# PaddlePaddle/PaddleRobotics

Measured on AMD Instinct MI355X. Metric: env-steps/sec, 4096 A1 quadrupeds; 1/2/4/8-GPU scaling, higher is better.
Workload: dtype f32

## Files before the change

paddlerobotics_amd/csrc/etg_core16.h:

```cpp
#pragma once

#include <type_traits>

#include "etg_core.h"

namespace etg {

template <class Ctx, class = void> struct sweep_stream_ : std::false_type {};
template <class Ctx> struct sweep_stream_<Ctx, std::void_t<decltype(Ctx::kSweepStream)>> : std::bool_constant<Ctx::kSweepStream> {};
template <class Ctx, class... Args> ETG_HD void run_sweep_stream_(const Ctx& c, Args&&... args) { c.pgs_body_stream(args...); }
template <class Ctx, class = void> struct gram_mfma_ : std::false_type {};
template <class Ctx> struct gram_mfma_<Ctx, std::void_t<decltype(Ctx::kGramMfma)>> : std::bool_constant<Ctx::kGramMfma> {};

template <class F> struct State16 {
  V3<F> p;
  F qx, qy, qz, qw;
  V3<F> wb, vb;
  F q, qd;
  F lam;
  F contact;
  F energy;
  int sweeps;
};

template <class F, class Ctx> ETG_HD State16<F> load_state16(const Ctx& c, const float* base, const float* leg) {
  State16<F> L;
  L.p = {c.ld_env(base, BS_PX), c.ld_env(base, BS_PY), c.ld_env(base, BS_PZ)};
  L.qx = c.ld_env(base, BS_QX); L.qy = c.ld_env(base, BS_QY); L.qz = c.ld_env(base, BS_QZ); L.qw = c.ld_env(base, BS_QW);
  L.wb = {c.ld_env(base, BS_WX), c.ld_env(base, BS_WY), c.ld_env(base, BS_WZ)};
  L.vb = {c.ld_env(base, BS_VX), c.ld_env(base, BS_VY), c.ld_env(base, BS_VZ)};
  const F mj = c.jointf();
  L.q = mj * c.ld_joint(leg, LG_Q);
  L.qd = mj * c.ld_joint(leg, LG_QD);
  L.lam = c.ld_quad(leg, LG_LAM);
  L.contact = c.ld_legf(leg, LG_CONTACT);
// ... 252 lines not shown
    nwo = nw;
    const V t1w = {it1 * (one - nwx * nwx), -(it1 * (nwx * nwy)), -(it1 * (nwx * nwz))};
    const V t2w = {zero, it1 * nwz, -(it1 * nwy)};
    const auto s2 = c.sub_is(2);
    const V dw = {sel_(s1, t1w.x, sel_(s2, t2w.x, nw.x)), sel_(s1, t1w.y, sel_(s2, t2w.y, nw.y)), sel_(s1, t1w.z, sel_(s2, t2w.z, nw.z))};
    dn = {Rw.r0.x * nw.x + Rw.r1.x * nw.y + Rw.r2.x * nw.z, Rw.r0.y * nw.x + Rw.r1.y * nw.y + Rw.r2.y * nw.z,
          Rw.r0.z * nw.x + Rw.r1.z * nw.y + Rw.r2.z * nw.z};
    dir = {Rw.r0.x * dw.x + Rw.r1.x * dw.y + Rw.r2.x * dw.z, Rw.r0.y * dw.x + Rw.r1.y * dw.y + Rw.r2.y * dw.z,
           Rw.r0.z * dw.x + Rw.r1.z * dw.y + Rw.r2.z * dw.z};
  }
  auto act = phi < F(K.margin);
  const F rowf = (bodies ? one : mj) * sel_(act, one, zero) * live;
  V rc = pc - rad * dn;
  V k1 = cross(xax, rc - g.o1), k2 = cross(g.yax, rc - g.o2), k3 = cross(g.yax, rc - g.o3);
  if (knee) {
    if (Ctx::kFlat) dir = {sel_(s3, dn.x, dir.x), sel_(s3, dn.y, dir.y), sel_(s3, dn.z, dir.z)};
    const V rn = rad * dn;
    const V a12 = q12 - s12 * rn, a3 = ps_ - rn;
    const V b1 = cross(xax, a12 - s12 * g.o1), b2 = cross(g.yax, a12 - s12 * g.o2), b3 = bw1 * cross(g.yax, a3 - g.o3);
    k1 = {sel_(s3, b1.x, k1.x), sel_(s3, b1.y, k1.y), sel_(s3, b1.z, k1.z)};
    k2 = {sel_(s3, b2.x, k2.x), sel_(s3, b2.y, k2.y), sel_(s3, b2.z, k2.z)};
    k3 = {sel_(s3, b3.x, k3.x), sel_(s3, b3.y, k3.y), sel_(s3, b3.z, k3.z)};
  }
  const bool anyb = bodies && c.any_body((rowf * f3) > F(0.5f));
  F Jl0 = rowf * dot(dir, k1), Jl1 = rowf * dot(dir, k2), Jl2 = rowf * dot(dir, k3);
  F HJ0 = Hi11 * Jl0 + Hi12 * Jl1 + Hi13 * Jl2;
  F HJ1 = Hi12 * Jl0 + Hi22 * Jl1 + Hi23 * Jl2;
  F HJ2 = Hi13 * Jl0 + Hi23 * Jl1 + Hi33 * Jl2;
  W Jb = rowf * W{cross(rc, dir), dir};
  W G = Jb - (HJ0 * Fj[0] + HJ1 * Fj[1] + HJ2 * Fj[2]);
  F g6[6] = {G.a.x, G.a.y, G.a.z, G.l.x, G.l.y, G.l.z};
  fwd6(s, g6);
  const W sqv = {{sq[0], sq[1], sq[2]}, {sq[3], sq[4], sq[5]}};
  const W Zv = cmul(W{{g6[0], g6[1], g6[2]}, {g6[3], g6[4], g6[5]}}, sqv);
  F Z[6] = {Zv.a.x, Zv.a.y, Zv.a.z, Zv.l.x, Zv.l.y, Zv.l.z};
  c.phase(5);
  F lam = rowf * sel_(s0, F(K.warmstart), sel_(c.sub_is(3), F(K.warmstart_b), F(K.warmstart_t))) * L.lam;
  F hj[3] = {HJ0, HJ1, HJ2};
  constexpr bool gram = gram_mfma_<Ctx>::value;
  F A[4][3];
  F Akz[4] = {zero, zero, zero, zero};
  if constexpr (gram) {
    c.dpp_ready4(hj, &lam);
    typename Ctx::gram_t Af[4];
    c.gram16(Af, Z, Z);
#pragma unroll
    for (int lp = 0; lp < 4; lp++) {
// ... 127 lines not shown
    for (int k = 0; k < 6; k++) Z2[k] = comp(Z2v, k);
    const V vc2 = vbs + cross(wbs, rc2) + qs0 * kb1 + qs1 * kb2 + qs2 * kb3;
    u2s = rowf2 * dot(dir2, vc2);
    c.dpp_ready(Z2, 6);
    c.dpp_ready(hj2, 3);
    if constexpr (gram) {
      typename Ctx::gram_t Bf[4];
      c.gram16(Bf, Z, Z2);
#pragma unroll
      for (int lp = 0; lp < 4; lp++)
#pragma unroll
        for (int e = 0; e < 4; e++) BA[lp][e] = Bf[lp][e];
    }
#pragma unroll
    for (int lp = 0; lp < 4; lp++) {
#pragma unroll
      for (int e = 0; e < 4; e++) {
        if constexpr (!gram) {
          BA[lp][e] = c.rbcast(Z[0], 4 * lp + e) * Z2[0];
#pragma unroll
          for (int k = 1; k < 6; k++) c.fmac_rbcast(BA[lp][e], Z[k], Z2[k], 4 * lp + e);
        }
      }
#pragma unroll
      for (int t = 0; t < 2; t++) {
        BB[lp][t] = c.rbcast(Z2[0], 4 * lp + 1 + t) * Z2[0];
        AT[lp][t] = c.rbcast(Z2[0], 4 * lp + 1 + t) * Z[0];
#pragma unroll
        for (int k = 1; k < 6; k++) {
          c.fmac_rbcast(BB[lp][t], Z2[k], Z2[k], 4 * lp + 1 + t);
          c.fmac_rbcast(AT[lp][t], Z2[k], Z[k], 4 * lp + 1 + t);
        }
      }
    }
    F oa[4], ob[2], ot[2];
#pragma unroll
    for (int e = 0; e < 4; e++) oa[e] = c.qb(hj[0], e) * Jb0 + c.qb(hj[1], e) * Jb1 + c.qb(hj[2], e) * Jb2_;
#pragma unroll
    for (int t = 0; t < 2; t++) {
      ob[t] = c.qb(hj2[0], 1 + t) * Jb0 + c.qb(hj2[1], 1 + t) * Jb1 + c.qb(hj2[2], 1 + t) * Jb2_;
      ot[t] = c.qb(hj2[0], 1 + t) * Jl0 + c.qb(hj2[1], 1 + t) * Jl1 + c.qb(hj2[2], 1 + t) * Jl2;
    }
#pragma unroll
    for (int lp = 0; lp < 4; lp++) {
#pragma unroll
      for (int e = 0; e < 4; e++) BA[lp][e] = BA[lp][e] + ownl[lp] * oa[e];
#pragma unroll
      for (int t = 0; t < 2; t++) { BB[lp][t] = BB[lp][t] + ownl[lp] * ob[t]; AT[lp][t] = AT[lp][t] + ownl[lp] * ot[t]; }
    }
    F Add2 = hj2[0] * Jb0 + hj2[1] * Jb1 + hj2[2] * Jb2_;
    Add2 = Add2 + dot(Z2v, Z2v);
    iA2 = sel_(rowf2 > F(0.5f), rcp_(Add2), zero);
#pragma unroll
    for (int lp = 0; lp < 4; lp++) {
#pragma unroll
      for (int e = 0; e < 4; e++) { if (b_lds) c.slotb_st(4 * lp + e, BA[lp][e]); else sb[4 * lp + e] = BA[lp][e]; }
#pragma unroll
      for (int t = 0; t < 2; t++) {
        if (b_lds) { c.slotb_st(16 + 2 * lp + t, BB[lp][t]); c.slotb_st(24 + 2 * lp + t, AT[lp][t]); }
        else { sb[16 + 2 * lp + t] = BB[lp][t]; sb[24 + 2 * lp + t] = AT[lp][t]; }
      }
    }
    c.phase_p(12);
  }
  F sgn = zero, lamq = zero, iAq = zero, c0q = zero;
  F zj[6] = {zero, zero, zero, zero, zero, zero};
  if (joints) {
    F z6[6] = {P.a.x, P.a.y, P.a.z, P.l.x, P.l.y, P.l.z};
    fwd6(s, z6);
    const W zv = cmul(W{{z6[0], z6[1], z6[2]}, {z6[3], z6[4], z6[5]}}, sqv);
#pragma unroll
// ... 167 lines not shown
        const F lc = lam - u * iA;
        F dl;
        if (pyramid) {
          dl = fminf_(fmaxf_(lc, -lim), lim) - lam;
        } else {
          const F sq1 = lc * lc + F(1e-30f);
          const F sc = fminf_(one, lim * rsqrt_(sq1 + c.qswap12(sq1)));
          dl = lc * sc - lam;
        }
        dl = sel_(grip, dl, zero);
        const F b1 = c.rbcast(dl, 4 * lp + 1), b2 = c.rbcast(dl, 4 * lp + 2);
        u = u + A[lp][1] * b1 + A[lp][2] * b2;
        if (body) u2 = u2 + Bt[2 * lp] * b1 + Bt[2 * lp + 1] * b2;
        lam = lam + mt[lp] * dl;
      }
      if constexpr (body) body_friction(c.qb(lam, 3));
    };
    if constexpr (sweep_stream_<Ctx>::value && body && !joints && !pyramid) {
      if (K.res_thr > 0.0f) {
        F tol = F(K.res_sqrt) * iA, tol2 = F(K.res_sqrt) * iA2;
        c.opaque(tol); c.opaque(tol2);
        const unsigned cap = (unsigned)(K.iters > 1 ? K.iters : 1) - 1u;
        unsigned rem = cap;
        run_sweep_stream_(c, lam, u, u2, lam2, rem, iA, c0, tp.mu, A, Ak, mk0, mk3, mt, Bn, Bt, iA2, K.body_mu, ATr, BBr, tol, tol2);
        L.sweeps += (int)(cap - rem) + (rem != ~0u ? 1 : 0);
        return;
      }
    }
    if (K.res_thr > 0.0f) {
      F tol = F(K.res_sqrt) * iA, tol2 = F(K.res_sqrt) * iA2;
      if (body) { c.opaque(tol); c.opaque(tol2); }
      const F tolq = F(K.res_sqrt) * iAq;
      int it = 0;
      bool more;
      auto frozen = lam < lam;
      auto sweep_and_test = [&]() {
        const F lam0 = lam, u0 = u, lamq0 = lamq, lam20 = lam2, u20 = u2;
        pgs_sweep();
        it++;
        lam = sel_(frozen, lam0, lam);
        u = sel_(frozen, u0, u);
        if (joints) lamq = sel_(frozen, lamq0, lamq);
        auto moved = c.vote(fabsf_(lam - lam0) > tol);
        if (joints) moved = c.vote_or(moved, c.vote(fabsf_(lamq - lamq0) > tolq));
        if (body) {
          lam2 = sel_(frozen, lam20, lam2);
          u2 = sel_(frozen, u20, u2);
// ... 558 lines not shown
```

paddlerobotics_amd/csrc/etg_kernels.hip:

```cpp
#include <hip/hip_runtime.h>

#include <string>
#include <vector>

#include "etg_core16.h"
#include "gram16.h"
#include "policy_core.h"
#include "../../include/etgsim_step_policy.h"
#include "../../include/etgsim_collect.h"
#include "../../include/etgsim_monitor.h"
#include "../../include/etgsim_terminal.h"

#ifndef ETG_TU_PARTS
#define ETG_TU_PARTS 1
#define ETG_TU_PART 0
#endif
#define ETG_TU_HOST (ETG_TU_PART == 0)

namespace etg {

template <int CTRL> __device__ __forceinline__ float dpp_(float x) {
  return __int_as_float(__builtin_amdgcn_update_dpp(0, __float_as_int(x), CTRL, 0xF, 0xF, true));
}

// ... 573 lines not shown
  }
  __device__ __forceinline__ void fmac_rbcast12(float& acc, float x, const float* a) const {
#define ETG_L(R, N) "v_fmac_f32_dpp %0, %1, %" #N " row_newbcast:" #R " row_mask:0xf bank_mask:0xf bound_ctrl:1\n"
    asm(ETG_L(0, 2) ETG_L(1, 3) ETG_L(2, 4) ETG_L(4, 5) ETG_L(5, 6) ETG_L(6, 7) ETG_L(8, 8) ETG_L(9, 9) ETG_L(10, 10)
        ETG_L(12, 11) ETG_L(13, 12) ETG_L(14, 13)
        : "+&v"(acc)
        : "v"(x), "v"(a[0]), "v"(a[1]), "v"(a[2]), "v"(a[3]), "v"(a[4]), "v"(a[5]), "v"(a[6]), "v"(a[7]), "v"(a[8]), "v"(a[9]),
          "v"(a[10]), "v"(a[11]));
#undef ETG_L
  }
  __device__ __forceinline__ float row2_velocity(float acc, float x, const float* a, float y, const float* b) const {
    float p1 = 0.0f, p2 = 0.0f, p3 = 0.0f;
#define ETG_L(ACC, SRC, R, N) "v_fmac_f32_dpp %" #ACC ", %" #SRC ", %" #N " row_newbcast:" #R " row_mask:0xf bank_mask:0xf bound_ctrl:1\n"
    asm(ETG_L(0, 4, 0, 6) ETG_L(1, 4, 1, 7) ETG_L(2, 4, 2, 8) ETG_L(3, 4, 3, 9) ETG_L(0, 4, 4, 10) ETG_L(1, 4, 5, 11) ETG_L(2, 4, 6, 12) ETG_L(3, 4, 7, 13)
        ETG_L(0, 4, 8, 14) ETG_L(1, 4, 9, 15) ETG_L(2, 4, 10, 16) ETG_L(3, 4, 11, 17) ETG_L(0, 4, 12, 18) ETG_L(1, 4, 13, 19) ETG_L(2, 4, 14, 20) ETG_L(3, 4, 15, 21)
        ETG_L(0, 5, 1, 22) ETG_L(1, 5, 2, 23) ETG_L(2, 5, 5, 24) ETG_L(3, 5, 6, 25) ETG_L(0, 5, 9, 26) ETG_L(1, 5, 10, 27) ETG_L(2, 5, 13, 28) ETG_L(3, 5, 14, 29)
        : "+&v"(acc), "+&v"(p1), "+&v"(p2), "+&v"(p3)
        : "v"(x), "v"(y), "v"(a[0]), "v"(a[1]), "v"(a[2]), "v"(a[3]), "v"(a[4]), "v"(a[5]), "v"(a[6]), "v"(a[7]), "v"(a[8]), "v"(a[9]),
          "v"(a[10]), "v"(a[11]), "v"(a[12]), "v"(a[13]), "v"(a[14]), "v"(a[15]), "v"(b[0]), "v"(b[1]), "v"(b[2]), "v"(b[3]), "v"(b[4]),
          "v"(b[5]), "v"(b[6]), "v"(b[7]));
#undef ETG_L
    return (acc + p1) + (p2 + p3);
  }
#undef ETG_FMAC_DPP
#define ETG_DPPC " row_mask:0xf bank_mask:0xf bound_ctrl:1\n"
  __device__ __forceinline__ void pgs_normals(float& lam, float& u, float iA, float c0, const float (&A)[4][3], const float* mk0) const {
    float t, d;
#define ETG_ROW(LP, AOP, MOP)                                                    \
    "v_fma_f32 %[t], -%[u], %[iA], %[c0]\n"         \
    "v_max_f32_e64 %[d], -%[lam], %[t]\n"           \
    "v_fmac_f32_e32 %[lam], %[" MOP "], %[d]\n"     \
    "s_nop 0\n"                                                                    \
    "v_fmac_f32_dpp %[u], %[d], %[" AOP "] row_newbcast:" #LP ETG_DPPC
    asm(ETG_ROW(0, "a0", "m0") ETG_ROW(4, "a1", "m1") ETG_ROW(8, "a2", "m2") ETG_ROW(12, "a3", "m3")
        : [lam] "+&v"(lam), [u] "+&v"(u), [t] "=&v"(t), [d] "=&v"(d)
        : [iA] "v"(iA), [c0] "v"(c0), [a0] "v"(A[0][0]), [a1] "v"(A[1][0]), [a2] "v"(A[2][0]), [a3] "v"(A[3][0]),
          [m0] "v"(mk0[0]), [m1] "v"(mk0[1]), [m2] "v"(mk0[2]), [m3] "v"(mk0[3]));
  }
  __device__ __forceinline__ void pgs_normals_body(float& lam, float& u, float iA, float c0, const float (&A)[4][3], const float* Ak,
                                                   const float* mk0, const float* mk3) const {
    float t, d;
    asm(ETG_ROW(0, "a0", "m0") ETG_ROW(4, "a1", "m1") ETG_ROW(8, "a2", "m2") ETG_ROW(12, "a3", "m3")
        ETG_ROW(3, "k0", "n0") ETG_ROW(7, "k1", "n1") ETG_ROW(11, "k2", "n2") ETG_ROW(15, "k3", "n3")
        : [lam] "+&v"(lam), [u] "+&v"(u), [t] "=&v"(t), [d] "=&v"(d)
        : [iA] "v"(iA), [c0] "v"(c0), [a0] "v"(A[0][0]), [a1] "v"(A[1][0]), [a2] "v"(A[2][0]), [a3] "v"(A[3][0]),
          [m0] "v"(mk0[0]), [m1] "v"(mk0[1]), [m2] "v"(mk0[2]), [m3] "v"(mk0[3]),
// ... 90 lines not shown
        "v_fmaak_f32 %[sq], %[lc], %[lc], 0x0da24260\n"                                                 \
        "s_nop 1\n"                                                                                     \
        "v_add_f32_dpp %[sq], %[sq], %[sq] quad_perm:[0,2,1,3]" ETG_DPPC                                \
        "v_rsq_f32_e32 %[sq], %[sq]\n"                                                                  \
        "s_nop 0\n"                                                                                     \
        "v_mul_f32_e32 %[sc], %[lim], %[sq]\n"                                                          \
        "v_min_f32_e32 %[sc], 1.0, %[sc]\n"                                                             \
        "v_fma_f32 %[dl], %[lc], %[sc], -%[lam]\n"                                                      \
        "v_fmac_f32_e32 %[lam], %[mk], %[dl]\n"                                                         \
        "s_nop 0\n"                                                                                     \
        "v_fmac_f32_dpp %[u], %[dl], %[at0] row_newbcast:" #R1 ETG_DPPC                                 \
        "v_fmac_f32_dpp %[u2], %[dl], %[bb0] row_newbcast:" #R1 ETG_DPPC                                \
        "v_fmac_f32_dpp %[u], %[dl], %[at1] row_newbcast:" #R2 ETG_DPPC                                 \
        "v_fmac_f32_dpp %[u2], %[dl], %[bb1] row_newbcast:" #R2 ETG_DPPC                                \
        : [lam] "+&v"(lam2), [u2] "+&v"(u2), [u] "+&v"(u), [lc] "=&v"(lc), [sq] "=&v"(sq), [sc] "=&v"(sc), [dl] "=&v"(dl)           \
        : [iA] "v"(iA), [lim] "v"(lim), [at0] "v"(at0), [at1] "v"(at1), [bb0] "v"(bb0), [bb1] "v"(bb1), [mk] "v"(mk))
    switch (lp) { case 0: ETG_PAIRB(1, 2); break; case 1: ETG_PAIRB(5, 6); break; case 2: ETG_PAIRB(9, 10); break; default: ETG_PAIRB(13, 14); break; }
#undef ETG_PAIRB
  }
#ifndef ETG_NO_ASM_SWEEP
  __device__ __forceinline__ void pgs_body_stream(float& lam, float& u, float& u2, float& lam2, unsigned& rem, float iA, float c0, float mue,
                                                  const float (&A)[4][3], const float* Ak, const float* mk0, const float* mk3, const float* mt,
                                                  const float* bn, const float* bt, float iA2, float body_mu, const float (&AT)[4][2],
                                                  const float (&BB)[4][2], float tol, float tol2) const {
    const unsigned row16 = 0xFFFFu << (tid & 16);
    const unsigned fl = (tid & 32) ? 0u : row16, fh = (tid & 32) ? row16 : 0u;
    float w, wu, wu2, w2, t, dA, dB, lnq, lbn, iAg, limg, lim, lc, sq, sc, iA2g, lim2g, rr;
    unsigned x, gm, tmp;
    unsigned long long live, mv, sa;
#define ETG_SGM "s_or_b32 %[gm], vcc_lo, vcc_hi\n"
#define ETG_SU2(D, LP, BOP) "v_fmac_f32_dpp %[wu2], %[" D "], %[" BOP "] row_newbcast:" #LP ETG_DPPC
#define ETG_SROW(D, LP, AOP, MOP, FILL)                                              \
    "v_fma_f32 %[t], -%[wu], %[iA], %[c0]\n"                                         \
    "v_max_f32_e64 %[" D "], -%[w], %[t]\n"                                          \
    "v_fmac_f32_e32 %[w], %[" MOP "], %[" D "]\n"                                    \
    FILL                                                                             \
    "v_fmac_f32_dpp %[wu], %[" D "], %[" AOP "] row_newbcast:" #LP ETG_DPPC
#define ETG_SPAIR(D, R1, R2, A1, A2, MOP, F1, F2, F3)                                \
    "v_fma_f32 %[lc], -%[wu], %[iAg], %[w]\n"                                        \
    "v_fmaak_f32 %[sq], %[lc], %[lc], 0x0da24260\n"                                  \
    F1                                                                               \
    "v_add_f32_dpp %[sq], %[sq], %[sq] quad_perm:[0,2,1,3]" ETG_DPPC                 \
    "v_rsq_f32_e32 %[sq], %[sq]\n"                                                   \
    F2                                                                               \
    "v_mul_f32_e32 %[sc], %[limg], %[sq]\n"                                          \
    "v_min_f32_e32 %[sc], 1.0, %[sc]\n"                                              \
    "v_fma_f32 %[" D "], %[lc], %[sc], -%[w]\n"                                      \
    "v_fmac_f32_e32 %[w], %[" MOP "], %[" D "]\n"                                    \
    F3                                                                               \
    "v_fmac_f32_dpp %[wu], %[" D "], %[" A1 "] row_newbcast:" #R1 ETG_DPPC           \
    "v_fmac_f32_dpp %[wu], %[" D "], %[" A2 "] row_newbcast:" #R2 ETG_DPPC
#define ETG_SLEG(LP, LEGBITS, R1, R2, MOP)                                           \
    "s_and_b32 %[tmp], %[gm], " LEGBITS "\n"                                         \
    "s_cbranch_scc0 .Letg_sw_leg" #LP "_%=\n"                                        \
    "v_fma_f32 %[lc], -%[wu2], %[iA2g], %[w2]\n"                                     \
    "v_fmaak_f32 %[sq], %[lc], %[lc], 0x0da24260\n"                                  \
    "s_nop 1\n"                                                                      \
    "v_add_f32_dpp %[sq], %[sq], %[sq] quad_perm:[0,2,1,3]" ETG_DPPC                 \
    "v_rsq_f32_e32 %[sq], %[sq]\n"                                                   \
    "s_nop 0\n"                                                                      \
    "v_mul_f32_e32 %[sc], %[lim2g], %[sq]\n"                                         \
    "v_min_f32_e32 %[sc], 1.0, %[sc]\n"                                              \
    "v_fma_f32 %[dA], %[lc], %[sc], -%[w2]\n"                                        \
    "v_fmac_f32_e32 %[w2], %[" MOP "], %[dA]\n"                                      \
    "s_nop 0\n"                                                                      \
    "v_fmac_f32_dpp %[wu], %[dA], %[at" #LP "0] row_newbcast:" #R1 ETG_DPPC          \
    "v_fmac_f32_dpp %[wu2], %[dA], %[bb" #LP "0] row_newbcast:" #R1 ETG_DPPC         \
    "v_fmac_f32_dpp %[wu], %[dA], %[at" #LP "1] row_newbcast:" #R2 ETG_DPPC          \
    "v_fmac_f32_dpp %[wu2], %[dA], %[bb" #LP "1] row_newbcast:" #R2 ETG_DPPC         \
    ".Letg_sw_leg" #LP "_%=:\n"
    asm volatile(
        "s_mov_b64 vcc, -1\n"
        ".Letg_sw_top_%=:\n"
        "v_mov_b32_e32 %[wu2], %[u2]\n"
        "v_fma_f32 %[t], -%[u], %[iA], %[c0]\n"
        "v_max_f32_e64 %[dA], -%[lam], %[t]\n"
        "v_fma_f32 %[w], %[m0], %[dA], %[lam]\n"
        "v_mov_b32_e32 %[wu], %[u]\n"
        "v_fmac_f32_dpp %[wu], %[dA], %[a0] row_newbcast:0" ETG_DPPC
        ETG_SROW("dB", 4, "a1", "m1", ETG_SU2("dA", 0, "b0"))
        ETG_SROW("dA", 8, "a2", "m2", ETG_SU2("dB", 4, "b1"))
        ETG_SROW("dB", 12, "a3", "m3", ETG_SU2("dA", 8, "b2"))
        ETG_SROW("dA", 3, "k0", "n0", ETG_SU2("dB", 12, "b3"))
        ETG_SROW("dB", 7, "k1", "n1", ETG_SU2("dA", 3, "b4"))
        ETG_SROW("dA", 11, "k2", "n2", ETG_SU2("dB", 7, "b5"))
        ETG_SROW("dB", 15, "k3", "n3", ETG_SU2("dA", 11, "b6"))
        ETG_SU2("dB", 15, "b7")
        "v_mov_b32_dpp %[lnq], %[w] quad_perm:[0,0,0,0]" ETG_DPPC
        "v_mov_b32_dpp %[lbn], %[w] quad_perm:[3,3,3,3]" ETG_DPPC
        "v_cmp_lt_f32_e64 %[sa], 0, %[lnq]\n"
        "v_mul_f32_e32 %[lim], %[mue], %[lnq]\n"
        "v_cndmask_b32_e64 %[iAg], 0, %[iA], %[sa]\n"
        "v_cndmask_b32_e64 %[limg], %[big], %[lim], %[sa]\n"
        ETG_SPAIR("dA", 1, 2, "a01", "a02", "t0",
                  "v_and_b32_e32 %[x], vcc_lo, %[fl]\n" "v_and_or_b32 %[x], vcc_hi, %[fh], %[x]\n",
                  "v_cmp_ne_u32_e64 %[live], 0, %[x]\n",
                  "v_mov_b32_e32 %[w2], %[lam2]\n")
        ETG_SPAIR("dB", 5, 6, "a11", "a12", "t1", ETG_SU2("dA", 1, "e0") ETG_SU2("dA", 2, "e1"),
                  "v_cmp_lt_f32_e32 vcc, 0, %[lbn]\n",
                  "v_mul_f32_e32 %[lim], %[bmu], %[lbn]\n")
        ETG_SPAIR("dA", 9, 10, "a21", "a22", "t2", ETG_SU2("dB", 5, "e2") ETG_SU2("dB", 6, "e3"),
                  "v_cndmask_b32_e32 %[iA2g], 0, %[iA2], vcc\n",
                  "v_cndmask_b32_e32 %[lim2g], %[big], %[lim], vcc\n")
        ETG_SPAIR("dB", 13, 14, "a31", "a32", "t3", ETG_SU2("dA", 9, "e4") ETG_SU2("dA", 10, "e5"),
                  ETG_SGM,
                  "v_sub_f32_e32 %[rr], %[w], %[lam]\n")
        ETG_SU2("dB", 13, "e6") ETG_SU2("dB", 14, "e7")
        "v_cmp_gt_f32_e64 %[mv], |%[rr]|, %[tol]\n"
        "s_cbranch_scc0 .Letg_sw_nf_%=\n"
        ETG_SLEG(0, "0x000f000f", 1, 2, "t0")
        ETG_SLEG(1, "0x00f000f0", 5, 6, "t1")
        ETG_SLEG(2, "0x0f000f00", 9, 10, "t2")
        ETG_SLEG(3, "0xf000f000", 13, 14, "t3")
        "v_sub_f32_e32 %[rr], %[w2], %[lam2]\n"
        "v_cmp_gt_f32_e64 %[sa], |%[rr]|, %[tol2]\n"
        "s_or_b64 %[mv], %[mv], %[sa]\n"
        "v_cndmask_b32_e64 %[lam2], %[lam2], %[w2], %[live]\n"
        ".Letg_sw_nf_%=:\n"
        "v_cndmask_b32_e64 %[lam], %[lam], %[w], %[live]\n"
        "v_cndmask_b32_e64 %[u], %[u], %[wu], %[live]\n"
        "v_cndmask_b32_e64 %[u2], %[u2], %[wu2], %[live]\n"
        "s_and_b64 vcc, %[mv], %[live]\n"
        "s_cbranch_scc0 .Letg_sw_end_%=\n"
        "s_sub_u32 %[rem], %[rem], 1\n"
        "s_cbranch_scc0 .Letg_sw_top_%=\n"
        ".Letg_sw_end_%=:\n"
        : [lam] "+&v"(lam), [u] "+&v"(u), [u2] "+&v"(u2), [lam2] "+&v"(lam2), [rem] "+&s"(rem), [w] "=&v"(w), [wu] "=&v"(wu), [wu2] "=&v"(wu2),
          [w2] "=&v"(w2), [t] "=&v"(t), [dA] "=&v"(dA), [dB] "=&v"(dB), [lnq] "=&v"(lnq), [lbn] "=&v"(lbn), [iAg] "=&v"(iAg), [limg] "=&v"(limg),
          [lim] "=&v"(lim), [lc] "=&v"(lc), [sq] "=&v"(sq), [sc] "=&v"(sc), [iA2g] "=&v"(iA2g), [lim2g] "=&v"(lim2g), [rr] "=&v"(rr), [x] "=&v"(x),
          [gm] "=&s"(gm), [tmp] "=&s"(tmp), [live] "=&s"(live), [mv] "=&s"(mv), [sa] "=&s"(sa)
        : [iA] "v"(iA), [c0] "v"(c0), [mue] "v"(mue), [big] "v"(1e30f), [a0] "v"(A[0][0]), [a1] "v"(A[1][0]), [a2] "v"(A[2][0]), [a3] "v"(A[3][0]),
          [m0] "v"(mk0[0]), [m1] "v"(mk0[1]), [m2] "v"(mk0[2]), [m3] "v"(mk0[3]),
          [k0] "v"(Ak[0]), [k1] "v"(Ak[1]), [k2] "v"(Ak[2]), [k3] "v"(Ak[3]),
          [n0] "v"(mk3[0]), [n1] "v"(mk3[1]), [n2] "v"(mk3[2]), [n3] "v"(mk3[3]),
          [b0] "v"(bn[0]), [b1] "v"(bn[1]), [b2] "v"(bn[2]), [b3] "v"(bn[3]), [b4] "v"(bn[4]), [b5] "v"(bn[5]), [b6] "v"(bn[6]), [b7] "v"(bn[7]),
          [a01] "v"(A[0][1]), [a02] "v"(A[0][2]), [a11] "v"(A[1][1]), [a12] "v"(A[1][2]), [a21] "v"(A[2][1]), [a22] "v"(A[2][2]),
          [a31] "v"(A[3][1]), [a32] "v"(A[3][2]), [t0] "v"(mt[0]), [t1] "v"(mt[1]), [t2] "v"(mt[2]), [t3] "v"(mt[3]),
          [e0] "v"(bt[0]), [e1] "v"(bt[1]), [e2] "v"(bt[2]), [e3] "v"(bt[3]), [e4] "v"(bt[4]), [e5] "v"(bt[5]), [e6] "v"(bt[6]), [e7] "v"(bt[7]),
          [iA2] "v"(iA2), [bmu] "s"(body_mu), [at00] "v"(AT[0][0]), [at01] "v"(AT[0][1]), [at10] "v"(AT[1][0]), [at11] "v"(AT[1][1]),
          [at20] "v"(AT[2][0]), [at21] "v"(AT[2][1]), [at30] "v"(AT[3][0]), [at31] "v"(AT[3][1]),
          [bb00] "v"(BB[0][0]), [bb01] "v"(BB[0][1]), [bb10] "v"(BB[1][0]), [bb11] "v"(BB[1][1]),
          [bb20] "v"(BB[2][0]), [bb21] "v"(BB[2][1]), [bb30] "v"(BB[3][0]), [bb31] "v"(BB[3][1]),
          [tol] "v"(tol), [tol2] "v"(tol2), [fl] "v"(fl), [fh] "v"(fh)
        : "vcc", "scc");
#undef ETG_SGM
#undef ETG_SU2
#undef ETG_SROW
#undef ETG_SPAIR
#undef ETG_SLEG
  }
#endif
#undef ETG_DPPC
  __device__ __forceinline__ void dpp_ready10(float* z, float* hj, float* lam) const {
    asm volatile("s_nop 1" : "+v"(z[0]), "+v"(z[1]), "+v"(z[2]), "+v"(z[3]), "+v"(z[4]), "+v"(z[5]), "+v"(hj[0]), "+v"(hj[1]), "+v"(hj[2]), "+v"(lam[0]));
  }
  __device__ __forceinline__ static int slotb_field(int k) { return k < 30 ? PR_LINK + k : PR_KP + (k - 30); }
  __device__ __forceinline__ void slotb_st(int k, float v) const { const_cast<float*>(lds)[slotb_field(k) * 64] = v; }
  __device__ __forceinline__ float slotb_ld(int k) const { return lds[slotb_field(k) * 64]; }
  __device__ __forceinline__ void opaque(float& v) const { asm volatile("" : "+v"(v)); }
  __device__ __forceinline__ void opaque3(float* v) const { asm volatile("" : "+v"(v[0]), "+v"(v[1]), "+v"(v[2])); }
  __device__ __forceinline__ void dpp_ready(float* v, int n) const {
    if (n == 6) asm volatile("s_nop 1" : "+v"(v[0]), "+v"(v[1]), "+v"(v[2]), "+v"(v[3]), "+v"(v[4]), "+v"(v[5]));
    else if (n == 3) asm volatile("s_nop 1" : "+v"(v[0]), "+v"(v[1]), "+v"(v[2]));
    else asm volatile("s_nop 1" : "+v"(v[0]));
  }
  __device__ __forceinline__ float ld_joint(const float* p, int f0) const { return p[(size_t)(f0 + sc) * NL + col]; }
  __device__ __forceinline__ void st_joint(float* p, int f0, float v) const { if (gate && sub < 3) p[(size_t)(f0 + sub) * NL + col] = v; }
  __device__ __forceinline__ float ld_quad(const float* p, int f0) const { return p[(size_t)(f0 + sub) * NL + col]; }
  __device__ __forceinline__ void st_quad(float* p, int f0, float v) const { if (gate) p[(size_t)(f0 + sub) * NL + col] = v; }
  __device__ __forceinline__ float ld_legf(const float* p, int f) const { return p[(size_t)f * NL + col]; }
  __device__ __forceinline__ void st_legf(float* p, int f, float v) const { if (gate && sub == 0) p[(size_t)f * NL + col] = v; }
  __device__ __forceinline__ float ld_env(const float* p, int f) const { return p[(size_t)f * N + env]; }
// ... 33 lines not shown
    if (K.terrain == 0) { h = 0.0f; nx = 0.0f; ny = 0.0f; nz = 1.0f; }
    else heightfield_query(K, env, x, y, h, nx, ny, nz);
  }
  __device__ __forceinline__ void terrain_fetch(const KCfg& K, float x, float y, float* tap) const { heightfield_fetch(K, env, x, y, tap); }
  __device__ __forceinline__ void terrain_finish(const KCfg& K, const float* tap, float& h, float& nx, float& ny, float& nz) const {
    heightfield_finish(K, tap, h, nx, ny, nz);
  }
};
template <bool FLAT, bool KNEE = false, bool PLAIN = false, bool SLOTB_LDS = false> struct GpuCtx16T : GpuCtx16 {
  static constexpr bool kFlat = FLAT;
  static constexpr bool kKnee = KNEE;
  static constexpr bool kPlain = PLAIN;
  static constexpr bool kSlotBLds = SLOTB_LDS;
  static constexpr bool kStepLocal = false;
#ifdef ETG_NO_ASM_SWEEP
  static constexpr bool kAsmSweep = false;
#else
  static constexpr bool kAsmSweep = true;
#endif
#ifdef ETG_GRAM_DPP
  static constexpr bool kGramMfma = false;
#else
  static constexpr bool kGramMfma = true;
#endif
#ifdef ETG_NO_ASM_SWEEP
  static constexpr bool kSweepStream = false;
#else
  static constexpr bool kSweepStream = true;
#endif
};

template <bool FLAT, bool KNEE, bool PLAIN> struct GpuCtx16W : GpuCtx16T<FLAT, KNEE, PLAIN> {
  static constexpr bool kStepLocal = true;
  __device__ __forceinline__ float tpar(int k) const { return this->lds[k * 64]; }
  __device__ __forceinline__ float tpar_joint(int base) const { return this->lds[(base + this->sc) * 64]; }
  __device__ __forceinline__ float tpar_link(int k) const { return this->sub < 3 ? this->lds[(PR_LINK + 10 * this->sub + k) * 64] : 0.0f; }
};
constexpr int PARK16 = 36;
__device__ __forceinline__ void park16(float* p, const State16<float>& L, const StepCtl16<float>& S) {
  const float v[PARK16] = {L.p.x, L.p.y, L.p.z, L.qx, L.qy, L.qz, L.qw, L.wb.x, L.wb.y, L.wb.z, L.vb.x, L.vb.y, L.vb.z, L.q, L.qd, L.lam, L.contact,
                           __int_as_float(S.step_count), __int_as_float(S.tick), __int_as_float(S.has_last), S.last, S.lbx, S.lby, S.lbz, S.last_fwx,
                           S.ret, S.len, S.r0, S.r1, S.r2, S.fx0, S.fx1, S.fy0, S.fy1, 0.0f, 0.0f};
#pragma unroll
  for (int k = 0; k < PARK16; k++) p[k * 64] = v[k];
}
__device__ __forceinline__ void unpark16(const float* p, State16<float>& L, StepCtl16<float>& S) {
// ... 2098 lines not shown
```

Before: 48.17 million.

## Skip body-contact Gram columns and sweep rows for legs without active body contacts

Computes a per-wave body-contact mask and builds the body-coupling Gram columns (BB/AT) only for legs whose body rows are active, using a DPP asm path that branches over inactive legs. The streamed PGS sweep is specialised so that when only one leg has body contacts, a dedicated loop variant with a single body row and pair runs instead of all four. This cuts DPP multiply-accumulate work in setup and in every sweep iteration, at the cost of more code size, more branches, and added dependence on the mask logic (helpers such as body_mask, mask_any and mask_leg) being correct.

New measurement: 48.13 million, median of 3. Within noise of the previous version (-0.1%).

```diff
diff --git a/paddlerobotics_amd/csrc/etg_core16.h b/paddlerobotics_amd/csrc/etg_core16.h
--- a/paddlerobotics_amd/csrc/etg_core16.h
+++ b/paddlerobotics_amd/csrc/etg_core16.h
@@ -3,6 +3,10 @@
 #include <type_traits>
 
 #include "etg_core.h"
+
+#ifdef ETG_TEST_DROP_BODY_LEG
+extern "C" { inline int etg_test_drop_body_leg = -1; }
+#endif
 
 namespace etg {
 
@@ -11,6 +15,10 @@
 template <class Ctx, class... Args> ETG_HD void run_sweep_stream_(const Ctx& c, Args&&... args) { c.pgs_body_stream(args...); }
 template <class Ctx, class = void> struct gram_mfma_ : std::false_type {};
 template <class Ctx> struct gram_mfma_<Ctx, std::void_t<decltype(Ctx::kGramMfma)>> : std::bool_constant<Ctx::kGramMfma> {};
+
+template <class Ctx, class = void> struct leg_cols_ : std::false_type {};
+template <class Ctx> struct leg_cols_<Ctx, std::void_t<decltype(Ctx::kLegCols)>> : std::bool_constant<Ctx::kLegCols> {};
+template <class Ctx, class... Args> ETG_HD void run_leg_cols_(const Ctx& c, Args&&... args) { c.leg_cols(args...); }
 
 template <class F> struct State16 {
   V3<F> p;
@@ -309,7 +317,15 @@
     k2 = {sel_(s3, b2.x, k2.x), sel_(s3, b2.y, k2.y), sel_(s3, b2.z, k2.z)};
     k3 = {sel_(s3, b3.x, k3.x), sel_(s3, b3.y, k3.y), sel_(s3, b3.z, k3.z)};
   }
+#ifdef ETG_BODY_ALL_LEGS
   const bool anyb = bodies && c.any_body((rowf * f3) > F(0.5f));
+#else
+  auto bm = c.body_mask((rowf * f3) > F(0.5f));
+#ifdef ETG_TEST_DROP_BODY_LEG
+  if (etg_test_drop_body_leg >= 0) bm &= ~decltype(bm)(0x000F000F000F000Full << (4 * etg_test_drop_body_leg));
+#endif
+  const bool anyb = bodies && c.mask_any(bm);
+#endif
   F Jl0 = rowf * dot(dir, k1), Jl1 = rowf * dot(dir, k2), Jl2 = rowf * dot(dir, k3);
   F HJ0 = Hi11 * Jl0 + Hi12 * Jl1 + Hi13 * Jl2;
   F HJ1 = Hi12 * Jl0 + Hi22 * Jl1 + Hi23 * Jl2;
@@ -483,6 +499,7 @@
           for (int k = 1; k < 6; k++) c.fmac_rbcast(BA[lp][e], Z[k], Z2[k], 4 * lp + e);
         }
       }
+#ifdef ETG_BODY_ALL_LEGS
 #pragma unroll
       for (int t = 0; t < 2; t++) {
         BB[lp][t] = c.rbcast(Z2[0], 4 * lp + 1 + t) * Z2[0];
@@ -493,6 +510,7 @@
           c.fmac_rbcast(AT[lp][t], Z2[k], Z[k], 4 * lp + 1 + t);
         }
       }
+#endif
     }
     F oa[4], ob[2], ot[2];
 #pragma unroll
@@ -506,8 +524,30 @@
     for (int lp = 0; lp < 4; lp++) {
 #pragma unroll
       for (int e = 0; e < 4; e++) BA[lp][e] = BA[lp][e] + ownl[lp] * oa[e];
+#ifdef ETG_BODY_ALL_LEGS
 #pragma unroll
       for (int t = 0; t < 2; t++) { BB[lp][t] = BB[lp][t] + ownl[lp] * ob[t]; AT[lp][t] = AT[lp][t] + ownl[lp] * ot[t]; }
+#else
+      if constexpr (leg_cols_<Ctx>::value) {
+        run_leg_cols_(c, BB[lp], AT[lp], Z2, Z, ownl[lp], ob, ot, bm, lp);
+        continue;
+      }
+      BB[lp][0] = BB[lp][1] = AT[lp][0] = AT[lp][1] = zero;
+      if (c.mask_leg(bm, lp)) {
+#pragma unroll
+        for (int t = 0; t < 2; t++) {
+          BB[lp][t] = c.rbcast(Z2[0], 4 * lp + 1 + t) * Z2[0];
+          AT[lp][t] = c.rbcast(Z2[0], 4 * lp + 1 + t) * Z[0];
+#pragma unroll
+          for (int k = 1; k < 6; k++) {
+            c.fmac_rbcast(BB[lp][t], Z2[k], Z2[k], 4 * lp + 1 + t);
+            c.fmac_rbcast(AT[lp][t], Z2[k], Z[k], 4 * lp + 1 + t);
+          }
+        }
+#pragma unroll
+        for (int t = 0; t < 2; t++) { BB[lp][t] = BB[lp][t] + ownl[lp] * ob[t]; AT[lp][t] = AT[lp][t] + ownl[lp] * ot[t]; }
+      }
+#endif
     }
     F Add2 = hj2[0] * Jb0 + hj2[1] * Jb1 + hj2[2] * Jb2_;
     Add2 = Add2 + dot(Z2v, Z2v);
@@ -721,7 +761,11 @@
         c.opaque(tol); c.opaque(tol2);
         const unsigned cap = (unsigned)(K.iters > 1 ? K.iters : 1) - 1u;
         unsigned rem = cap;
+#ifdef ETG_BODY_ALL_LEGS
         run_sweep_stream_(c, lam, u, u2, lam2, rem, iA, c0, tp.mu, A, Ak, mk0, mk3, mt, Bn, Bt, iA2, K.body_mu, ATr, BBr, tol, tol2);
+#else
+        run_sweep_stream_(c, lam, u, u2, lam2, rem, iA, c0, tp.mu, A, Ak, mk0, mk3, mt, Bn, Bt, iA2, K.body_mu, ATr, BBr, tol, tol2, bm);
+#endif
         L.sweeps += (int)(cap - rem) + (rem != ~0u ? 1 : 0);
         return;
       }
diff --git a/paddlerobotics_amd/csrc/etg_kernels.hip b/paddlerobotics_amd/csrc/etg_kernels.hip
--- a/paddlerobotics_amd/csrc/etg_kernels.hip
+++ b/paddlerobotics_amd/csrc/etg_kernels.hip
@@ -619,6 +619,46 @@
 #undef ETG_L
     return (acc + p1) + (p2 + p3);
   }
+#ifndef ETG_BODY_ALL_LEGS
+  __device__ __forceinline__ void leg_cols(float (&bb)[2], float (&at)[2], const float* z2, const float* z, float ownl, const float* ob,
+                                           const float* ot, unsigned bm, int lp) const {
+    unsigned tmp;
+#define ETG_DPPB " row_mask:0xf bank_mask:0xf bound_ctrl:1\n"
+#define ETG_LK(OP, K, R1, R2)                                                       \
+    OP " %[bb0], %[p" #K "], %[p" #K "] row_newbcast:" #R1 ETG_DPPB                   \
+    OP " %[at0], %[p" #K "], %[z" #K "] row_newbcast:" #R1 ETG_DPPB                   \
+    OP " %[bb1], %[p" #K "], %[p" #K "] row_newbcast:" #R2 ETG_DPPB                   \
+    OP " %[at1], %[p" #K "], %[z" #K "] row_newbcast:" #R2 ETG_DPPB
+#define ETG_LEGCOLS(LEGBITS, R1, R2)                                                \
+    asm("v_mov_b32_e32 %[bb0], 0\n"                                                  \
+        "v_mov_b32_e32 %[at0], 0\n"                                                  \
+        "v_mov_b32_e32 %[bb1], 0\n"                                                  \
+        "v_mov_b32_e32 %[at1], 0\n"                                                  \
+        "s_and_b32 %[tmp], %[bm], " LEGBITS "\n"                                     \
+        "s_cbranch_scc0 .Letg_lc_end_%=\n"                                           \
+        ETG_LK("v_mul_f32_dpp", 0, R1, R2) ETG_LK("v_fmac_f32_dpp", 1, R1, R2) ETG_LK("v_fmac_f32_dpp", 2, R1, R2)                 \
+        ETG_LK("v_fmac_f32_dpp", 3, R1, R2) ETG_LK("v_fmac_f32_dpp", 4, R1, R2) ETG_LK("v_fmac_f32_dpp", 5, R1, R2)                \
+        "v_fmac_f32_e32 %[bb0], %[ownl], %[ob0]\n"                                   \
+        "v_fmac_f32_e32 %[at0], %[ownl], %[ot0]\n"                                   \
+        "v_fmac_f32_e32 %[bb1], %[ownl], %[ob1]\n"                                   \
+        "v_fmac_f32_e32 %[at1], %[ownl], %[ot1]\n"                                   \
+        ".Letg_lc_end_%=:\n"                                                         \
+        : [bb0] "=&v"(bb[0]), [bb1] "=&v"(bb[1]), [at0] "=&v"(at[0]), [at1] "=&v"(at[1]), [tmp] "=&s"(tmp)                         \
+        : [bm] "s"(bm), [p0] "v"(z2[0]), [p1] "v"(z2[1]), [p2] "v"(z2[2]), [p3] "v"(z2[3]), [p4] "v"(z2[4]), [p5] "v"(z2[5]),     \
+          [z0] "v"(z[0]), [z1] "v"(z[1]), [z2] "v"(z[2]), [z3] "v"(z[3]), [z4] "v"(z[4]), [z5] "v"(z[5]), [ownl] "v"(ownl),       \
+          [ob0] "v"(ob[0]), [ob1] "v"(ob[1]), [ot0] "v"(ot[0]), [ot1] "v"(ot[1])                                                   \
+        : "scc")
+    switch (lp) {
+      case 0: ETG_LEGCOLS("0x000f000f", 1, 2); break;
+      case 1: ETG_LEGCOLS("0x00f000f0", 5, 6); break;
+      case 2: ETG_LEGCOLS("0x0f000f00", 9, 10); break;
+      default: ETG_LEGCOLS("0xf000f000", 13, 14); break;
+    }
+#undef ETG_LEGCOLS
+#undef ETG_LK
+#undef ETG_DPPB
+  }
+#endif
 #undef ETG_FMAC_DPP
 #define ETG_DPPC " row_mask:0xf bank_mask:0xf bound_ctrl:1\n"
   __device__ __forceinline__ void pgs_normals(float& lam, float& u, float iA, float c0, const float (&A)[4][3], const float* mk0) const {
@@ -755,7 +795,11 @@
   __device__ __forceinline__ void pgs_body_stream(float& lam, float& u, float& u2, float& lam2, unsigned& rem, float iA, float c0, float mue,
                                                   const float (&A)[4][3], const float* Ak, const float* mk0, const float* mk3, const float* mt,
                                                   const float* bn, const float* bt, float iA2, float body_mu, const float (&AT)[4][2],
-                                                  const float (&BB)[4][2], float tol, float tol2) const {
+                                                  const float (&BB)[4][2], float tol, float tol2
+#ifndef ETG_BODY_ALL_LEGS
+                                                  , unsigned bm
+#endif
+                                                  ) const {
     const unsigned row16 = 0xFFFFu << (tid & 16);
     const unsigned fl = (tid & 32) ? 0u : row16, fh = (tid & 32) ? row16 : 0u;
     float w, wu, wu2, w2, t, dA, dB, lnq, lbn, iAg, limg, lim, lc, sq, sc, iA2g, lim2g, rr;
@@ -786,6 +830,9 @@
 #define ETG_SLEG(LP, LEGBITS, R1, R2, MOP)                                           \
     "s_and_b32 %[tmp], %[gm], " LEGBITS "\n"                                         \
     "s_cbranch_scc0 .Letg_sw_leg" #LP "_%=\n"                                        \
+    ETG_SLEGPAIR(LP, R1, R2, MOP)                                                    \
+    ".Letg_sw_leg" #LP "_%=:\n"
+#define ETG_SLEGPAIR(LP, R1, R2, MOP)                                                \
     "v_fma_f32 %[lc], -%[wu2], %[iA2g], %[w2]\n"                                     \
     "v_fmaak_f32 %[sq], %[lc], %[lc], 0x0da24260\n"                                  \
     "s_nop 1\n"                                                                      \
@@ -800,63 +847,87 @@
     "v_fmac_f32_dpp %[wu], %[dA], %[at" #LP "0] row_newbcast:" #R1 ETG_DPPC          \
     "v_fmac_f32_dpp %[wu2], %[dA], %[bb" #LP "0] row_newbcast:" #R1 ETG_DPPC         \
     "v_fmac_f32_dpp %[wu], %[dA], %[at" #LP "1] row_newbcast:" #R2 ETG_DPPC          \
-    "v_fmac_f32_dpp %[wu2], %[dA], %[bb" #LP "1] row_newbcast:" #R2 ETG_DPPC         \
-    ".Letg_sw_leg" #LP "_%=:\n"
+    "v_fmac_f32_dpp %[wu2], %[dA], %[bb" #LP "1] row_newbcast:" #R2 ETG_DPPC
+#define ETG_SLOOP(V, BROWS, BPAIRS, TAIL)                                            \
+        ".Letg_sw_top" V "_%=:\n"                                                    \
+              \
+        "v_mov_b32_e32 %[wu2], %[u2]\n"                                              \
+        "v_fma_f32 %[t], -%[u], %[iA], %[c0]\n"                                      \
+        "v_max_f32_e64 %[dA], -%[lam], %[t]\n"                                       \
+        "v_fma_f32 %[w], %[m0], %[dA], %[lam]\n"                      \
+        "v_mov_b32_e32 %[wu], %[u]\n"                                                \
+        "v_fmac_f32_dpp %[wu], %[dA], %[a0] row_newbcast:0" ETG_DPPC                 \
+        ETG_SROW("dB", 4, "a1", "m1", ETG_SU2("dA", 0, "b0"))                        \
+        ETG_SROW("dA", 8, "a2", "m2", ETG_SU2("dB", 4, "b1"))                        \
+        ETG_SROW("dB", 12, "a3", "m3", ETG_SU2("dA", 8, "b2"))                       \
+        BROWS                                                                        \
+         \
+        "v_mov_b32_dpp %[lnq], %[w] quad_perm:[0,0,0,0]" ETG_DPPC                    \
+        "v_mov_b32_dpp %[lbn], %[w] quad_perm:[3,3,3,3]" ETG_DPPC                    \
+        "v_cmp_lt_f32_e64 %[sa], 0, %[lnq]\n"                                        \
+        "v_mul_f32_e32 %[lim], %[mue], %[lnq]\n"                                     \
+        "v_cndmask_b32_e64 %[iAg], 0, %[iA], %[sa]\n"                                \
+        "v_cndmask_b32_e64 %[limg], %[big], %[lim], %[sa]\n"                         \
+         \
+        ETG_SPAIR("dA", 1, 2, "a01", "a02", "t0",                                    \
+                  "v_and_b32_e32 %[x], vcc_lo, %[fl]\n" "v_and_or_b32 %[x], vcc_hi, %[fh], %[x]\n", \
+                  "v_cmp_ne_u32_e64 %[live], 0, %[x]\n",                             \
+                  "v_mov_b32_e32 %[w2], %[lam2]\n")                                  \
+        ETG_SPAIR("dB", 5, 6, "a11", "a12", "t1", ETG_SU2("dA", 1, "e0") ETG_SU2("dA", 2, "e1"), \
+                  "v_cmp_lt_f32_e32 vcc, 0, %[lbn]\n",                               \
+                  "v_mul_f32_e32 %[lim], %[bmu], %[lbn]\n")                          \
+        ETG_SPAIR("dA", 9, 10, "a21", "a22", "t2", ETG_SU2("dB", 5, "e2") ETG_SU2("dB", 6, "e3"), \
+                  "v_cndmask_b32_e32 %[iA2g], 0, %[iA2], vcc\n",                     \
+                  "v_cndmask_b32_e32 %[lim2g], %[big], %[lim], vcc\n")               \
+        ETG_SPAIR("dB", 13, 14, "a31", "a32", "t3", ETG_SU2("dA", 9, "e4") ETG_SU2("dA", 10, "e5"), \
+                  ETG_SGM,                                                           \
+                  "v_sub_f32_e32 %[rr], %[w], %[lam]\n")                             \
+        ETG_SU2("dB", 13, "e6") ETG_SU2("dB", 14, "e7")                              \
+        "v_cmp_gt_f32_e64 %[mv], |%[rr]|, %[tol]\n"                                  \
+        "s_cbranch_scc0 .Letg_sw_nf" V "_%=\n"                        \
+                         \
+        BPAIRS                                                                       \
+        "v_sub_f32_e32 %[rr], %[w2], %[lam2]\n"                                      \
+        "v_cmp_gt_f32_e64 %[sa], |%[rr]|, %[tol2]\n"                                 \
+        "s_or_b64 %[mv], %[mv], %[sa]\n"                                             \
+        "v_cndmask_b32_e64 %[lam2], %[lam2], %[w2], %[live]\n"                       \
+        ".Letg_sw_nf" V "_%=:\n"                                                     \
+         \
+        "v_cndmask_b32_e64 %[lam], %[lam], %[w], %[live]\n"                          \
+        "v_cndmask_b32_e64 %[u], %[u], %[wu], %[live]\n"                             \
+        "v_cndmask_b32_e64 %[u2], %[u2], %[wu2], %[live]\n"                          \
+        "s_and_b64 vcc, %[mv], %[live]\n"                                            \
+        "s_cbranch_scc0 .Letg_sw_end_%=\n"                            \
+        "s_sub_u32 %[rem], %[rem], 1\n"                                              \
+        "s_cbranch_scc0 .Letg_sw_top" V "_%=\n"                       \
+        TAIL
+#define ETG_SBROWS_ALL                                                               \
+        ETG_SROW("dA", 3, "k0", "n0", ETG_SU2("dB", 12, "b3"))                       \
+        ETG_SROW("dB", 7, "k1", "n1", ETG_SU2("dA", 3, "b4"))                        \
+        ETG_SROW("dA", 11, "k2", "n2", ETG_SU2("dB", 7, "b5"))                       \
+        ETG_SROW("dB", 15, "k3", "n3", ETG_SU2("dA", 11, "b6"))                      \
+        ETG_SU2("dB", 15, "b7")
+#define ETG_SBPAIRS_ALL                                                              \
+        ETG_SLEG(0, "0x000f000f", 1, 2, "t0")                                        \
+        ETG_SLEG(1, "0x00f000f0", 5, 6, "t1")                                        \
+        ETG_SLEG(2, "0x0f000f00", 9, 10, "t2")                                       \
+        ETG_SLEG(3, "0xf000f000", 13, 14, "t3")
+#define ETG_SBROWS_ONE(R, AOP, MOP, BOP) ETG_SROW("dA", R, AOP, MOP, ETG_SU2("dB", 12, "b3")) ETG_SU2("dA", R, BOP)
     asm volatile(
         "s_mov_b64 vcc, -1\n"
-        ".Letg_sw_top_%=:\n"
-        "v_mov_b32_e32 %[wu2], %[u2]\n"
-        "v_fma_f32 %[t], -%[u], %[iA], %[c0]\n"
-        "v_max_f32_e64 %[dA], -%[lam], %[t]\n"
-        "v_fma_f32 %[w], %[m0], %[dA], %[lam]\n"
-        "v_mov_b32_e32 %[wu], %[u]\n"
-        "v_fmac_f32_dpp %[wu], %[dA], %[a0] row_newbcast:0" ETG_DPPC
-        ETG_SROW("dB", 4, "a1", "m1", ETG_SU2("dA", 0, "b0"))
-        ETG_SROW("dA", 8, "a2", "m2", ETG_SU2("dB", 4, "b1"))
-        ETG_SROW("dB", 12, "a3", "m3", ETG_SU2("dA", 8, "b2"))
-        ETG_SROW("dA", 3, "k0", "n0", ETG_SU2("dB", 12, "b3"))
-        ETG_SROW("dB", 7, "k1", "n1", ETG_SU2("dA", 3, "b4"))
-        ETG_SROW("dA", 11, "k2", "n2", ETG_SU2("dB", 7, "b5"))
-        ETG_SROW("dB", 15, "k3", "n3", ETG_SU2("dA", 11, "b6"))
-        ETG_SU2("dB", 15, "b7")
-        "v_mov_b32_dpp %[lnq], %[w] quad_perm:[0,0,0,0]" ETG_DPPC
-        "v_mov_b32_dpp %[lbn], %[w] quad_perm:[3,3,3,3]" ETG_DPPC
-        "v_cmp_lt_f32_e64 %[sa], 0, %[lnq]\n"
-        "v_mul_f32_e32 %[lim], %[mue], %[lnq]\n"
-        "v_cndmask_b32_e64 %[iAg], 0, %[iA], %[sa]\n"
-        "v_cndmask_b32_e64 %[limg], %[big], %[lim], %[sa]\n"
-        ETG_SPAIR("dA", 1, 2, "a01", "a02", "t0",
-                  "v_and_b32_e32 %[x], vcc_lo, %[fl]\n" "v_and_or_b32 %[x], vcc_hi, %[fh], %[x]\n",
-                  "v_cmp_ne_u32_e64 %[live], 0, %[x]\n",
-                  "v_mov_b32_e32 %[w2], %[lam2]\n")
-        ETG_SPAIR("dB", 5, 6, "a11", "a12", "t1", ETG_SU2("dA", 1, "e0") ETG_SU2("dA", 2, "e1"),
-                  "v_cmp_lt_f32_e32 vcc, 0, %[lbn]\n",
-                  "v_mul_f32_e32 %[lim], %[bmu], %[lbn]\n")
-        ETG_SPAIR("dA", 9, 10, "a21", "a22", "t2", ETG_SU2("dB", 5, "e2") ETG_SU2("dB", 6, "e3"),
-                  "v_cndmask_b32_e32 %[iA2g], 0, %[iA2], vcc\n",
-                  "v_cndmask_b32_e32 %[lim2g], %[big], %[lim], vcc\n")
-        ETG_SPAIR("dB", 13, 14, "a31", "a32", "t3", ETG_SU2("dA", 9, "e4") ETG_SU2("dA", 10, "e5"),
-                  ETG_SGM,
-                  "v_sub_f32_e32 %[rr], %[w], %[lam]\n")
-        ETG_SU2("dB", 13, "e6") ETG_SU2("dB", 14, "e7")
-        "v_cmp_gt_f32_e64 %[mv], |%[rr]|, %[tol]\n"
-        "s_cbranch_scc0 .Letg_sw_nf_%=\n"
-        ETG_SLEG(0, "0x000f000f", 1, 2, "t0")
-        ETG_SLEG(1, "0x00f000f0", 5, 6, "t1")
-        ETG_SLEG(2, "0x0f000f00", 9, 10, "t2")
-        ETG_SLEG(3, "0xf000f000", 13, 14, "t3")
-        "v_sub_f32_e32 %[rr], %[w2], %[lam2]\n"
-        "v_cmp_gt_f32_e64 %[sa], |%[rr]|, %[tol2]\n"
-        "s_or_b64 %[mv], %[mv], %[sa]\n"
-        "v_cndmask_b32_e64 %[lam2], %[lam2], %[w2], %[live]\n"
-        ".Letg_sw_nf_%=:\n"
-        "v_cndmask_b32_e64 %[lam], %[lam], %[w], %[live]\n"
-        "v_cndmask_b32_e64 %[u], %[u], %[wu], %[live]\n"
-        "v_cndmask_b32_e64 %[u2], %[u2], %[wu2], %[live]\n"
-        "s_and_b64 vcc, %[mv], %[live]\n"
-        "s_cbranch_scc0 .Letg_sw_end_%=\n"
-        "s_sub_u32 %[rem], %[rem], 1\n"
-        "s_cbranch_scc0 .Letg_sw_top_%=\n"
+#ifdef ETG_BODY_ALL_LEGS
+        ETG_SLOOP("", ETG_SBROWS_ALL, ETG_SBPAIRS_ALL, "")
+#else
+        "s_andn2_b32 %[tmp], %[bm], 0x000f000f\n" "s_cbranch_scc0 .Letg_sw_top0_%=\n"
+        "s_andn2_b32 %[tmp], %[bm], 0x00f000f0\n" "s_cbranch_scc0 .Letg_sw_top1_%=\n"
+        "s_andn2_b32 %[tmp], %[bm], 0x0f000f00\n" "s_cbranch_scc0 .Letg_sw_top2_%=\n"
+        "s_andn2_b32 %[tmp], %[bm], 0xf000f000\n" "s_cbranch_scc0 .Letg_sw_top3_%=\n"
+        ETG_SLOOP("", ETG_SBROWS_ALL, ETG_SBPAIRS_ALL, "s_branch .Letg_sw_end_%=\n")
+        ETG_SLOOP("0", ETG_SBROWS_ONE(3, "k0", "n0", "b4"), ETG_SLEGPAIR(0, 1, 2, "t0"), "s_branch .Letg_sw_end_%=\n")
+        ETG_SLOOP("1", ETG_SBROWS_ONE(7, "k1", "n1", "b5"), ETG_SLEGPAIR(1, 5, 6, "t1"), "s_branch .Letg_sw_end_%=\n")
+        ETG_SLOOP("2", ETG_SBROWS_ONE(11, "k2", "n2", "b6"), ETG_SLEGPAIR(2, 9, 10, "t2"), "s_branch .Letg_sw_end_%=\n")
+        ETG_SLOOP("3", ETG_SBROWS_ONE(15, "k3", "n3", "b7"), ETG_SLEGPAIR(3, 13, 14, "t3"), "")
+#endif
         ".Letg_sw_end_%=:\n"
         : [lam] "+&v"(lam), [u] "+&v"(u), [u2] "+&v"(u2), [lam2] "+&v"(lam2), [rem] "+&s"(rem), [w] "=&v"(w), [wu] "=&v"(wu), [wu2] "=&v"(wu2),
           [w2] "=&v"(w2), [t] "=&v"(t), [dA] "=&v"(dA), [dB] "=&v"(dB), [lnq] "=&v"(lnq), [lbn] "=&v"(lbn), [iAg] "=&v"(iAg), [limg] "=&v"(limg),
@@ -875,12 +946,20 @@
           [bb00] "v"(BB[0][0]), [bb01] "v"(BB[0][1]), [bb10] "v"(BB[1][0]), [bb11] "v"(BB[1][1]),
           [bb20] "v"(BB[2][0]), [bb21] "v"(BB[2][1]), [bb30] "v"(BB[3][0]), [bb31] "v"(BB[3][1]),
           [tol] "v"(tol), [tol2] "v"(tol2), [fl] "v"(fl), [fh] "v"(fh)
+#ifndef ETG_BODY_ALL_LEGS
+          , [bm] "s"(bm)
+#endif
         : "vcc", "scc");
 #undef ETG_SGM
 #undef ETG_SU2
 #undef ETG_SROW
 #undef ETG_SPAIR
 #undef ETG_SLEG
+#undef ETG_SLEGPAIR
+#undef ETG_SLOOP
+#undef ETG_SBROWS_ALL
+#undef ETG_SBPAIRS_ALL
+#undef ETG_SBROWS_ONE
   }
 #endif
 #undef ETG_DPPC
@@ -960,6 +1039,11 @@
   static constexpr bool kGramMfma = false;
 #else
   static constexpr bool kGramMfma = true;
+#endif
+#if defined(ETG_NO_ASM_SWEEP) || defined(ETG_BODY_ALL_LEGS)
+  static constexpr bool kLegCols = false;
+#else
+  static constexpr bool kLegCols = true;
 #endif
 #ifdef ETG_NO_ASM_SWEEP
   static constexpr bool kSweepStream = false;
```
